# GPUPeople/spECK

Measured on AMD Instinct MI355X. Metric: SpGEMM GFLOP/s (2*flops_intermediate/s), A*A, higher is better.
Workload: dtype f64; 1 GPU; scircuit-like A*A (SURVEY 8d stand-in); rows=170998, nnzA=965730, products=8470902, nnzC=5291656, parallelism=single

## Files before the change

### speck_amd/csrc/esc_rows.hpp

```cpp
#pragma once
#include <type_traits>

#include "device_common.hpp"
#include "launch.hpp"
#include "row_groups.hpp"
#include "esc.hpp"

namespace speck {

template <typename T>
using Acc = double;

template <typename T, u32 L>
constexpr u32 num_esc_group_lds()
{
    return 4u * L * (u32)sizeof(Acc<T>) + L * (4u + (u32)sizeof(Acc<T>));
}

template <typename T, u32 L>
__device__ __forceinline__ u32 num_esc_row(const SubWave<L>& g, unsigned char* mine, const ProductSrc<T>& src, u32 a0, u32 a1,
                                           u32* __restrict__ out_col, T* __restrict__ out_val, u32 room)
{
    static_assert(L == 8 || L == 16, "8 or 16 lanes per row");
    using Mask = typename std::conditional<L <= 8, u32, u64>::type;
    constexpr u32 PER = kEscPerLane, NP = PER * L, TAG = L == 8 ? 5u : 6u;
    Acc<T>* s_vals = reinterpret_cast<Acc<T>*>(mine);
    Acc<T>* s_av = s_vals + NP;
    u32* s_off = reinterpret_cast<u32*>(s_av + L);
    const u32 gl = g.lane;
    const bool have = a0 + gl < a1;
    uint2 sl = make_uint2(0u, 0u);
    Acc<T> av = 0;
    if (have) {
        sl = src.b_sl[a0 + gl];
        av = (Acc<T>)src.a_val[a0 + gl];
    }
    u32 total;
    const u32 incl = g.inclusive_scan(sl.y, &total, nullptr);
    const bool nonempty = sl.y != 0;
    const u32 before = (u32)__popcll(g.ballot(nonempty) & ((1ull << gl) - 1ull));
    if (nonempty) {
        s_off[before] = sl.x - (incl - sl.y);
        s_av[before] = av;
    }
    Mask ends;
    if constexpr (L == 8) {
        ends = esc_group_or((nonempty && incl < 32u) ? (1u << incl) : 0u);
    } else {
        const u64 bit = (nonempty && incl < 64u) ? (1ull << incl) : 0ull;
        ends = (u64(esc_row_or((u32)(bit >> 32))) << 32) | esc_row_or((u32)bit);
    }
    wave_lds_fence();
    u32 key[PER], c[PER];
    T bv[PER];
    Acc<T> a[PER];
#pragma unroll
    for (u32 u = 0; u < PER; ++u) {
        const u32 p = u * L + gl;
        c[u] = 0;
        bv[u] = T(0);
        a[u] = 0;
        if (p < total) {
            u32 j;
            if constexpr (L <= 8) j = (u32)__popc(ends & ((2u << p) - 1u));
            else j = (u32)__popcll(ends & ((2ull << p) - 1ull));
            const u32 ib = s_off[j] + p;
            c[u] = src.b_col[ib];
            bv[u] = src.b_val[ib];
            a[u] = s_av[j];
        }
    }
#pragma unroll
    for (u32 u = 0; u < PER; ++u) {
        const u32 p = u * L + gl;
        key[u] = kEscInvalid;
        if (p < total) {
            const T prod = (T)a[u] * bv[u];
            s_vals[p] = (Acc<T>)prod;
            key[u] = (c[u] << TAG) | p;
        }
    }
    wave_lds_fence();
    esc_sort<L>(key, gl);
    u32 col[PER];
    Acc<T> sum[PER];
#pragma unroll
    for (u32 r = 0; r < PER; ++r) {
        const bool valid = gl * PER + r < total;
        col[r] = valid ? key[r] >> TAG : kEscInvalid;
// ... 8 lines not shown
        sum[r] += same ? sum[r - 1] : Acc<T>(0);
    }
    const u32 prev_col = dpp_move<kDppRowShr + 1>(kEscInvalid, col[PER - 1]);
    const bool cont = gl != 0 && col[0] != kEscInvalid && prev_col == col[0];
    Acc<T> chain = sum[PER - 1];
    bool stop = !(lead[PER - 1] && cont);
#pragma unroll
    for (u32 d = 1; d < L; d <<= 1) {
        Acc<T> t;
        bool ts;
        if (d == 1) {
            t = dpp_move_f64<kDppRowShr + 1>(0.0, chain);
            ts = dpp_move<kDppRowShr + 1>(1u, (u32)stop) != 0;
        } else if (d == 2) {
            t = dpp_move_f64<kDppRowShr + 2>(0.0, chain);
            ts = dpp_move<kDppRowShr + 2>(1u, (u32)stop) != 0;
        } else if (d == 4) {
            t = dpp_move_f64<kDppRowShr + 4>(0.0, chain);
            ts = dpp_move<kDppRowShr + 4>(1u, (u32)stop) != 0;
        } else {
            t = dpp_move_f64<kDppRowShr + 8>(0.0, chain);
            ts = dpp_move<kDppRowShr + 8>(1u, (u32)stop) != 0;
        }
        const bool in_group = gl >= d;
        if (!stop && in_group) chain += t;
        stop = stop || !in_group || ts;
    }
    const Acc<T> from_prev = dpp_move_f64<kDppRowShr + 1>(0.0, chain);
    const Acc<T> carry = cont ? from_prev : Acc<T>(0);
#pragma unroll
    for (u32 r = 0; r < PER; ++r) sum[r] += lead[r] ? carry : Acc<T>(0);
    const u32 next_col = dpp_move<kDppRowShl + 1>(kEscInvalid, col[0]);
    bool tail[PER];
    u32 ntail = 0;
#pragma unroll
    for (u32 r = 0; r < PER; ++r) {
        const u32 after = r + 1 < PER ? col[r + 1] : (gl == L - 1 ? kEscInvalid : next_col);
        tail[r] = col[r] != kEscInvalid && after != col[r];
        ntail += tail[r] ? 1u : 0u;
    }
    u32 all;
    u32 pos = g.inclusive_scan(ntail, &all, nullptr) - ntail;
    const bool write = all <= room;
#pragma unroll
    for (u32 r = 0; r < PER; ++r)
        if (tail[r] && write) {
            out_col[pos] = col[r];
            out_val[pos] = (T)sum[r];
            ++pos;
        }
    wave_lds_fence();
    return all;
}

template <typename T, u32 L, int THREADS, bool FUSED = false>
__device__ __forceinline__ void num_esc_body(unsigned char* smem, const ProductSrc<T>& src, const RowWork& w,
                                             u32* __restrict__ c_col, T* __restrict__ c_val, int cls, u32 bidx,
                                             u32 nblk, u32 hint = kNoCount, u32* __restrict__ counts = nullptr)
{
    using G = SubWave<L>;
    constexpr u32 NG = THREADS / L;
    const G g;
    const u32 gid = threadIdx.x / L;
    unsigned char* mine = smem + gid * num_esc_group_lds<T, L>();
    RowCursor cur = open_list<FUSED>(w, cls, hint, bidx, nblk, NG, gid, (w.xcd_aware & 8u) != 0);
    if (wave_void(cur.miss)) return;
    while (cur.more()) {
        const RowRec rec = cur.take();
        u32 place = rec.base, room = 0xFFFFFFFFu;
        if constexpr (FUSED) {
            place = w.nf_pred_off[rec.row];
            room = w.nf_pred_off[rec.row + 1] - place;
        }
        const u32 all = num_esc_row<T, L>(g, mine, src, rec.a0, rec.a1, c_col + place, c_val + place, room);
        if constexpr (FUSED) {
            if (g.lane == 0) {
                counts[rec.row] = all;
                if (all != room) const_cast<DeviceStats*>(w.st)->capacity_miss = 1;
            }
        }
    }
}

}
```

### speck_amd/csrc/esc_wide.hpp

```cpp
#pragma once
#include <type_traits>

#include "device_common.hpp"
#include "launch.hpp"
#include "row_groups.hpp"
#include "esc.hpp"
#include "esc_rows.hpp"

namespace speck {

constexpr int kDppRowRor8 = 0x128, kDppWaveShl1 = 0x130, kDppWaveShr1 = 0x138;

template <u32 M>
__device__ __forceinline__ u32 fetch_xor(u32 v)
{
    if constexpr (M == 1) return dpp_fetch<kDppQuadXor1>(v);
    else if constexpr (M == 2) return dpp_fetch<kDppQuadXor2>(v);
    else if constexpr (M == 3) return dpp_fetch<kDppQuadMirror>(v);
    else if constexpr (M == 4) return esc_xor4(v);
    else if constexpr (M == 7) return dpp_fetch<kDppRowHalfMirror>(v);
    else if constexpr (M == 8) return dpp_fetch<kDppRowRor8>(v);
    else {
        static_assert(M == 15, "lane masks inside a DPP row");
        return dpp_fetch<kDppRowMirror>(v);
// ... 59 lines not shown

template <u32 L>
__device__ __forceinline__ void esc_sort_wide(u32 (&x)[4], u32 gl)
{
    static_assert(L == 32 || L == 64, "32 or 64 lanes per row");
    esc_sort64(x, gl & 15u);
    esc_merge_stage<7>(x, gl);
    if constexpr (L == 64) esc_merge_stage<8>(x, gl);
}

template <int CTRL>
__device__ __forceinline__ double wave_move_f64(double fill, double v)
{
    return dpp_move_f64<CTRL>(fill, v);
}

template <u32 L>
struct EscEnds {
    static constexpr u32 NP = 4u * L, NW = NP / 32u;
    uint2* pref;
    template <class G>
    __device__ __forceinline__ void build(const G& g, bool nonempty, u32 incl) const
    {
        if (g.lane < NW) pref[g.lane].x = 0u;
        wave_lds_fence();
        if (nonempty && incl < NP) atomicOr(&pref[incl >> 5].x, 1u << (incl & 31u));
        wave_lds_fence();
        const u32 w = g.lane < NW ? pref[g.lane].x : 0u;
        const u32 pc = (u32)__popc(w);
        u32 total;
        const u32 inc = g.inclusive_scan(pc, &total, nullptr);
        if (g.lane < NW) pref[g.lane].y = inc - pc;
        wave_lds_fence();
    }
    __device__ __forceinline__ u32 owner(u32 p) const
    {
        const uint2 e = pref[p >> 5];
        return e.y + (u32)__popc(e.x & ((2u << (p & 31u)) - 1u));
    }
};

template <typename T, u32 L>
constexpr u32 num_escw_group_lds()
{
    return 4u * L * (u32)sizeof(Acc<T>) + L * ((u32)sizeof(Acc<T>) + 4u) + (4u * L / 32u) * 8u;
}
template <u32 L>
constexpr u32 sym_escw_group_lds()
{
    return L * 4u + (4u * L / 32u) * 8u;
}

template <typename T, u32 L>
__device__ __forceinline__ u32 num_escw_row(const SubWave<L>& g, unsigned char* mine, const ProductSrc<T>& src, u32 a0, u32 a1,
                                            u32 cmin, u32* __restrict__ out_col, T* __restrict__ out_val, u32 room)
{
    static_assert(L == 32 || L == 64, "32 or 64 lanes per row");
    constexpr u32 PER = kEscPerLane, NP = PER * L, TAG = L == 32 ? 7u : 8u;
    static_assert((1u << TAG) == NP, "the product number fills the tag");
    static_assert(TAG + (L == 32 ? kNumEsc32RangeBits : kNumEsc64RangeBits) == 32, "key = column offset << TAG | product");
    Acc<T>* s_vals = reinterpret_cast<Acc<T>*>(mine);
    Acc<T>* s_av = s_vals + NP;
    u32* s_off = reinterpret_cast<u32*>(s_av + L);
    const EscEnds<L> ends{reinterpret_cast<uint2*>(s_off + L)};
    const u32 gl = g.lane;
    const bool have = a0 + gl < a1;
    uint2 sl = make_uint2(0u, 0u);
    Acc<T> av = 0;
    if (have) {
        sl = src.b_sl[a0 + gl];
        av = (Acc<T>)src.a_val[a0 + gl];
    }
    u32 total;
    const u32 incl = g.inclusive_scan(sl.y, &total, nullptr);
    const bool nonempty = sl.y != 0;
    const u32 before = (u32)__popcll(g.ballot(nonempty) & ((1ull << gl) - 1ull));
    if (nonempty) {
        s_off[before] = sl.x - (incl - sl.y);
        s_av[before] = av;
    }
    ends.build(g, nonempty, incl);
    u32 key[PER], c[PER];
    T bv[PER];
    Acc<T> a[PER];
#pragma unroll
    for (u32 u = 0; u < PER; ++u) {
        const u32 p = u * L + gl;
        c[u] = 0;
        bv[u] = T(0);
        a[u] = 0;
        if (p < total) {
            const u32 j = ends.owner(p);
            const u32 ib = s_off[j] + p;
            c[u] = src.b_col[ib];
            bv[u] = src.b_val[ib];
            a[u] = s_av[j];
        }
    }
#pragma unroll
    for (u32 u = 0; u < PER; ++u) {
        const u32 p = u * L + gl;
        key[u] = kEscInvalid;
        if (p < total) {
            const T prod = (T)a[u] * bv[u];
            s_vals[p] = (Acc<T>)prod;
            key[u] = ((c[u] - cmin) << TAG) | p;
        }
    }
    wave_lds_fence();
    esc_sort_wide<L>(key, gl);
    u32 col[PER];
    Acc<T> sum[PER];
#pragma unroll
    for (u32 r = 0; r < PER; ++r) {
        const bool valid = gl * PER + r < total;
        col[r] = valid ? key[r] >> TAG : kEscInvalid;
        sum[r] = valid ? s_vals[key[r] & (NP - 1u)] : Acc<T>(0);
    }
    bool lead[PER];
    lead[0] = true;
#pragma unroll
    for (u32 r = 1; r < PER; ++r) {
        const bool same = col[r] == col[r - 1] && col[r] != kEscInvalid;
        lead[r] = lead[r - 1] && same;
        sum[r] += same ? sum[r - 1] : Acc<T>(0);
// ... 10 lines not shown
        const bool take = !stop && rl >= D_;                                     \
        chain += take ? t : Acc<T>(0);                                           \
        stop = take ? ts : stop;                                                 \
    }
    SPECK_SEG_ROW(1)
    SPECK_SEG_ROW(2)
    SPECK_SEG_ROW(4)
    SPECK_SEG_ROW(8)
#undef SPECK_SEG_ROW
    {
        const Acc<T> t = __longlong_as_double(
            (u64(dpp_move<kDppRowBcast15, 0xA>(0u, (u32)(__double_as_longlong(chain) >> 32))) << 32) |
            dpp_move<kDppRowBcast15, 0xA>(0u, (u32)__double_as_longlong(chain)));
        const bool ts = dpp_move<kDppRowBcast15, 0xA>(1u, (u32)stop) != 0;
        const bool take = !stop && (gl & 16u) != 0;
        chain += take ? t : Acc<T>(0);
        stop = take ? ts : stop;
    }
    if constexpr (L == 64) {
        const Acc<T> t = __longlong_as_double(
            (u64(dpp_move<kDppRowBcast31, 0xC>(0u, (u32)(__double_as_longlong(chain) >> 32))) << 32) |
            dpp_move<kDppRowBcast31, 0xC>(0u, (u32)__double_as_longlong(chain)));
        const bool ts = dpp_move<kDppRowBcast31, 0xC>(1u, (u32)stop) != 0;
        const bool take = !stop && (gl & 32u) != 0;
        chain += take ? t : Acc<T>(0);
        stop = take ? ts : stop;
    }
    const Acc<T> from_prev = wave_move_f64<kDppWaveShr1>(0.0, chain);
    const Acc<T> carry = cont ? from_prev : Acc<T>(0);
#pragma unroll
    for (u32 r = 0; r < PER; ++r) sum[r] += lead[r] ? carry : Acc<T>(0);
    const u32 next_col = dpp_move<kDppWaveShl1>(kEscInvalid, col[0]);
    bool tail[PER];
    u32 ntail = 0;
#pragma unroll
    for (u32 r = 0; r < PER; ++r) {
        const u32 after = r + 1 < PER ? col[r + 1] : (gl == L - 1 ? kEscInvalid : next_col);
        tail[r] = col[r] != kEscInvalid && after != col[r];
        ntail += tail[r] ? 1u : 0u;
    }
    u32 all;
    u32 pos = g.inclusive_scan(ntail, &all, nullptr) - ntail;
    const bool write = all <= room;
#pragma unroll
    for (u32 r = 0; r < PER; ++r)
        if (tail[r] && write) {
            out_col[pos] = col[r] + cmin;
            out_val[pos] = (T)sum[r];
            ++pos;
        }
    wave_lds_fence();
    return all;
}

template <typename T, u32 L, int THREADS, bool FUSED = false>
__device__ __forceinline__ void num_escw_body(unsigned char* smem, const ProductSrc<T>& src, const RowWork& w,
                                              u32* __restrict__ c_col, T* __restrict__ c_val, int cls, u32 bidx,
                                              u32 nblk, u32 hint = kNoCount, u32* __restrict__ counts = nullptr)
{
    using G = SubWave<L>;
    constexpr u32 NG = THREADS / L;
    const G g;
    const u32 gid = threadIdx.x / L;
    unsigned char* mine = smem + gid * num_escw_group_lds<T, L>();
    RowCursor cur = open_list<FUSED>(w, cls, hint, bidx, nblk, NG, gid, (w.xcd_aware & 8u) != 0);
    if (wave_void(cur.miss)) return;
    while (cur.more()) {
        const RowRec rec = cur.take();
        u32 place = rec.base, room = 0xFFFFFFFFu;
        if constexpr (FUSED) {
            place = w.nf_pred_off[rec.row];
            room = w.nf_pred_off[rec.row + 1] - place;
        }
        const u32 all = num_escw_row<T, L>(g, mine, src, rec.a0, rec.a1, rec.cmin, c_col + place, c_val + place, room);
        if constexpr (FUSED) {
            if (g.lane == 0) {
                counts[rec.row] = all;
                if (all != room) const_cast<DeviceStats*>(w.st)->capacity_miss = 1;
            }
        }
    }
}

template <u32 L, int THREADS>
__device__ __forceinline__ void sym_escw_body(unsigned char* smem, const ProductSrc<float>& src, const RowWork& w,
                                              u32* __restrict__ counts, int cls, u32 bidx, u32 nblk,
                                              u32 hint = kNoCount)
{
    static_assert(L == 32 || L == 64, "32 or 64 lanes per row");
    using G = SubWave<L>;
    constexpr u32 NG = THREADS / L, PER = kEscPerLane;
    const G g;
    const u32 gid = threadIdx.x / L;
    u32* s_off = reinterpret_cast<u32*>(smem + gid * sym_escw_group_lds<L>());
    const EscEnds<L> ends{reinterpret_cast<uint2*>(s_off + L)};
    RowCursor cur = open_list<true>(w, cls, hint, bidx, nblk, NG, gid, (w.xcd_aware & 8u) != 0);
    if (wave_void(cur.miss)) return;
    const u32 gl = g.lane;
    while (cur.more()) {
        const RowRec rec = cur.take();
        uint2 sl = make_uint2(0u, 0u);
        if (rec.a0 + gl < rec.a1) sl = src.b_sl[rec.a0 + gl];
        u32 total;
        const u32 incl = g.inclusive_scan(sl.y, &total, nullptr);
        const bool nonempty = sl.y != 0;
        const u32 before = (u32)__popcll(g.ballot(nonempty) & ((1ull << gl) - 1ull));
        if (nonempty) s_off[before] = sl.x - (incl - sl.y);
        ends.build(g, nonempty, incl);
        u32 col[PER];
#pragma unroll
        for (u32 u = 0; u < PER; ++u) {
            const u32 p = u * L + gl;
            col[u] = kEscInvalid;
            if (p < total) col[u] = src.b_col[s_off[ends.owner(p)] + p];
        }
        esc_sort_wide<L>(col, gl);
        const u32 prev_col = dpp_move<kDppWaveShr1>(kEscInvalid, col[PER - 1]);
        u32 heads = 0;
#pragma unroll
        for (u32 r = 0; r < PER; ++r) {
            const u32 before_col = r ? col[r - 1] : (gl ? prev_col : kEscInvalid);
            heads += (col[r] != kEscInvalid && col[r] != before_col) ? 1u : 0u;
        }
        heads = g.reduce_add(heads, nullptr);
        if (gl == 0) store_row_count(w, counts, rec.row, heads);
        wave_lds_fence();
    }
}

}
```

### speck_amd/csrc/launch.hpp

```cpp
#pragma once
#include <hip/hip_ext.h>

#include "chain.hpp"
#include "device_common.hpp"

namespace speck {

u32 analysis_blocks(u32 m);
void set_analysis_wide_rows(u32 avg_len);
u32 scan_tiles(u32 m);

constexpr u32 kListRegions = (((u32)SYM_CLASSES > (u32)NUM_CLASSES ? (u32)SYM_CLASSES : (u32)NUM_CLASSES) + 1u) / 2u;
__host__ __device__ inline size_t class_list_records(u32 m) { return size_t(kListRegions) * (m ? m : 1u); }
template <typename Rec>
__host__ __device__ __forceinline__ Rec* class_rec_at(Rec* lists, u32 m, u32 cls, u32 i)
{
    return two_sided_at(lists, m, cls, i);
}

void launch_analysis(hipStream_t s, const u32* a_ro, const u32* a_col, const u32* b_ro, const u32* b_col, u32 m, u64 nnz_a,
                     u32* row_ops, u32* row_max_ops, u32* row_col_min, u32* row_col_max, u8* sym_cls, u32* counts,
                     RowRec* sym_recs, DeviceStats* st, const ClassifyParams& cp, uint2* b_sl, const Chain& chain,
                     u64* nf_off = nullptr, u64 expect_nf = ~0ull, u32 b_rows = ~0u,
                     u32* a_ro_copy = nullptr ,
// ... 213 lines not shown
void note_launch_status(hipError_t e, const char* what);
int take_launch_error();
#define SPECK_LAUNCH(kernel_, ...)                                          \
    do {                                                                    \
        hipLaunchKernelGGL(kernel_, __VA_ARGS__);                           \
        ::speck::note_launch_status(hipGetLastError(), #kernel_);           \
    } while (0)
#define SPECK_LAUNCH_TIMED(kernel_, grid_, block_, lds_, stream_, e0_, e1_, ...)                            \
    do {                                                                                                   \
        if (e0_) hipExtLaunchKernelGGL(kernel_, grid_, block_, lds_, stream_, e0_, e1_, 0, __VA_ARGS__);   \
        else hipLaunchKernelGGL(kernel_, grid_, block_, lds_, stream_, __VA_ARGS__);                       \
        ::speck::note_launch_status(hipGetLastError(), #kernel_);                                          \
    } while (0)

template <typename T>
void launch_numeric(hipStream_t s, int cls, u32 count, const CsrView<T>& A, const CsrView<T>& B,
                    const RowWork& w, u32* c_col, T* c_val, int cu_count);

template <typename T>
void launch_walk(hipStream_t s, const WalkArgs& args, const ProductSrc<T>& src, const Chain& chain, hipEvent_t e0 = nullptr,
                 hipEvent_t e1 = nullptr);

u32 grid_for(u32 count, u32 lds, int threads, int cu_count, u32 rows_per_block);

template <typename K>
void set_dyn_lds(K kernel, u32 bytes)
{
    if (bytes > 48 * 1024)
        note_launch_status(hipFuncSetAttribute(reinterpret_cast<const void*>(kernel),
                                               hipFuncAttributeMaxDynamicSharedMemorySize, (int)bytes),
                           "hipFuncSetAttribute(MaxDynamicSharedMemorySize)");
}

template <size_t N, typename LdsFn>
bool plan_light(const ClassSlot (&tab)[N], u32 mask, const u32* counts_hint, bool exact, int cu_count, LdsFn&& class_lds,
                u32 extra, hipStream_t s, hipEvent_t e0, hipEvent_t e1, ClassGrid* cg, u32* lds)
{
    *lds = 0;
    for (const ClassSlot& t : tab)
        if (mask >> t.cls & 1u) *lds = *lds > class_lds(t.cls) ? *lds : class_lds(t.cls);
    *cg = ClassGrid{};
    for (size_t k = 0; k < N; ++k) {
        const u32 hint = counts_hint[tab[k].cls];
        const bool on = (mask >> tab[k].cls & 1u) && hint;
        cg->first[k + 1] = cg->first[k] + (on ? grid_for(hint, *lds, 256, cu_count, tab[k].rows) : 0u);
        cg->cnt[k] = exact ? hint : kNoCount;
    }
    cg->first[N + 1] = cg->first[N] + extra;
    if (cg->first[N + 1] != 0) return true;
    if (e0) (void)hipEventRecord(e0, s), (void)hipEventRecord(e1, s);
    return false;
}
void set_grid_rounds(u32 block_classes, u32 subwave_classes);
void set_b8k_full_first(u32 mask);
void set_scan_small_items(int items);
void set_spill_big_grid(u32 blocks);

u32 symbolic_lds_bytes(int cls);
u32 numeric_lds_bytes(int cls, u32 vsize);

}
```

### speck_amd/csrc/numeric.hip

```cpp
#include <algorithm>
#include <type_traits>

#include "chain3.hpp"
#include "device_common.hpp"
#include "launch.hpp"
#include "row_groups.hpp"
#include "esc_rows.hpp"
#include "esc_wide.hpp"

namespace speck {

template <typename T, int THREADS>
constexpr u32 num_direct_lds()
{
    return THREADS * (12u + (u32)sizeof(T)) + (THREADS / 64 + 2 + win_words<Block<THREADS>>() + 3) / 4 * 16;
}

template <typename T, int THREADS>
__device__ __forceinline__ void num_direct_body(unsigned char* smem, const ProductSrc<T>& src, const RowWork& w,
                                                u32* __restrict__ c_col, T* __restrict__ c_val, u32 bidx,
                                                u32 nblk, u32 hint = kNoCount)
{
    using G = Block<THREADS>;
    const G g;
// ... 1552 lines not shown
void set_b8k_full_first(u32 mask) { g_b8k_full_first = mask; }
static u32 g_spill_big_grid = 256;
void set_spill_big_grid(u32 blocks) { g_spill_big_grid = blocks ? blocks : 256u; }

template <typename T, bool VERIFY>
static void launch_b8k(hipStream_t s, u32 count, const ProductSrc<T>& A, const u32* B, const RowWork& w, u32* c_col,
                       T* c_val, int cu_count)
{
    constexpr int cls = NUM_B8K;
    if (w.sliced) {
        const u32 sl = num_sliced_lds(num_group_lds<Block<256>, T, kNumB2KCap, 256>());
        SPECK_LAUNCH((num_sliced_kernel<T, VERIFY>), dim3(grid_for(count, sl, 256, cu_count, 1)), dim3(256), sl, s, A, B, w,
                     c_col, c_val, cls);
        return;
    }
    const auto all = launch_num_hash<Block<512>, T, kNumB8KCap, kB8KW1, kNumB8KMaxNnz, SORT_BITMAP, 512, 0, VERIFY>;
    const auto upper = launch_num_hash<Block<512>, T, kNumB8KCap, kB8KW1, kNumB8KMaxNnz, SORT_BITMAP, 512, kNumB8KHalfMaxNnz, VERIFY>;
    const auto lower = launch_num_hash<Block<512>, T, kNumB8KCap / 2, kB8KW1, kNumB8KHalfMaxNnz, SORT_BITMAP, 512, 0, VERIFY>;
    if (count * 2 < (u32)cu_count) {
        all(s, cls, count, A, B, w, c_col, c_val, cu_count);
        return;
    }
    const bool full_first = (g_b8k_full_first & (VERIFY ? 2u : 1u)) != 0;
    if (full_first) upper(s, cls, count, A, B, w, c_col, c_val, cu_count);
    lower(s, cls, count, A, B, w, c_col, c_val, cu_count);
    if (!full_first) upper(s, cls, count, A, B, w, c_col, c_val, cu_count);
}

template <typename T, bool VERIFY>
static void launch_d2(hipStream_t s, u32 count, const ProductSrc<T>& A, const u32* B, const RowWork& w, u32* c_col,
                      T* c_val, int cu_count)
{
    auto k = num_dense_kernel<T, kNumD2Cols, 1024, VERIFY>;
    const u32 lds = numeric_lds_bytes_t<T>(NUM_D2);
    set_dyn_lds(k, lds);
    SPECK_LAUNCH(k, dim3(grid_for(count, lds, 1024, cu_count, 1)), dim3(1024), lds, s, A, B, w, c_col, c_val, (int)NUM_D2);
}

template <typename T>
void launch_numeric_light(hipStream_t s, const u32* counts_hint, u32 mask, const CsrView<T>& Av,
                          const CsrView<T>& Bv, const RowWork& w, u32* c_col, T* c_val, int cu_count, bool exact,
                          hipEvent_t e0, hipEvent_t e1)
{
    constexpr size_t NS = kNumLightSlots;
    const u32 off_blocks = w.off_n ? std::min<u32>((w.off_n + 2047u) / 2048u, 512u) : 0u;
    ClassGrid cg;
    u32 lds;
    if (!plan_light(kNumLight, mask, counts_hint, exact, cu_count, numeric_lds_bytes_t<T>, off_blocks, s, e0, e1, &cg, &lds)) return;
    const bool tiny_only = cg.first[kNumTinyFirst] == 0 && !w.verify_numeric && !w.off_n;
    const ProductSrc<T> src{w.b_sl, Av.data, Bv.col_ids, Bv.data, w.w_sl};
    bool with_esc = false;
    for (size_t k = 0; k < NS; ++k)
        if ((kNumEscMask >> kNumLight[k].cls & 1u) && cg.first[k + 1] != cg.first[k]) with_esc = true;
    if (w.verify_numeric)
        SPECK_LAUNCH_TIMED((num_light_kernel<T, false, true>), dim3(cg.first[NS + 1]), dim3(256), lds, s, e0, e1, src,
                           Av.row_offsets, w, c_col, c_val, cg);
    else if (!tiny_only && with_esc)
        SPECK_LAUNCH_TIMED((num_light_kernel<T, true>), dim3(cg.first[NS + 1]), dim3(256), lds, s, e0, e1, src, Av.row_offsets, w,
                           c_col, c_val, cg);
    else if (!tiny_only)
        SPECK_LAUNCH_TIMED((num_light_kernel<T, false>), dim3(cg.first[NS + 1]), dim3(256), lds, s, e0, e1, src, Av.row_offsets, w,
                           c_col, c_val, cg);
    else
        SPECK_LAUNCH_TIMED((num_tiny_kernel<T>), dim3(cg.first[NS]), dim3(256), lds, s, e0, e1, src, Av.row_offsets, w,
                           c_col, c_val, cg);
}

template <typename T>
void launch_numeric_first(hipStream_t s, u32 count, const CsrView<T>& Av, const CsrView<T>& Bv, const RowWork& w,
                          u32* counts, int cu_count, u32 wcols, hipEvent_t e0, hipEvent_t e1)
{
    if (count == 0) {
        if (e0) (void)hipEventRecord(e0, s), (void)hipEventRecord(e1, s);
        return;
    }
    const ProductSrc<T> src{w.b_sl, Av.data, Bv.col_ids, Bv.data, w.w_sl};
    wcols = wcols < 256u ? 256u : (wcols > kNumD1Cols ? kNumD1Cols : (wcols + 255u) & ~255u);
    const u32 lds = (wcols + 256) * (u32)sizeof(Acc<T>) + wcols +
                    (2 * 256 + 256 / 64 + 2 + win_words<Block<256>>() + 3) / 4 * 16;
    if (w.nf_pred_off) {
        set_dyn_lds((nf_dense_kernel<T, 256, true>), lds);
        SPECK_LAUNCH_TIMED((nf_dense_kernel<T, 256, true>), dim3(grid_for(count, lds, 256, cu_count, 1)), dim3(256), lds, s, e0,
                           e1, src, Av.row_offsets, w, counts, wcols);
        return;
    }
    set_dyn_lds((nf_dense_kernel<T, 256>), lds);
    SPECK_LAUNCH_TIMED((nf_dense_kernel<T, 256>), dim3(grid_for(count, lds, 256, cu_count, 1)), dim3(256), lds, s, e0, e1,
                       src, Av.row_offsets, w, counts, wcols);
}

template <typename T>
void launch_numeric(hipStream_t s, int cls, u32 count, const CsrView<T>& Av, const CsrView<T>& Bv,
                    const RowWork& w, u32* c_col, T* c_val, int cu_count)
{
    if (count == 0) return;
    const ProductSrc<T> A{w.b_sl, Av.data, Bv.col_ids, Bv.data, w.w_sl};
    const u32* B = Av.row_offsets;
    switch (cls) {
        case NUM_B8K:
            if (w.verify_numeric)
                launch_b8k<T, true>(s, count, A, B, w, c_col, c_val, cu_count);
            else
                launch_b8k<T, false>(s, count, A, B, w, c_col, c_val, cu_count);
            break;
        case NUM_D2:
            if (w.verify_numeric)
// ... 71 lines not shown
```

### speck_amd/csrc/pipeline.hip

```cpp
#include <hip/hip_runtime.h>

#include <algorithm>
#include <chrono>
#include <cstdio>
#include <cstdlib>
#include <cstring>
#include <string>
#include <vector>

#include "../../include/speck_c_api.h"
#include "chain3.hpp"
#include "host_common.hpp"
#include "launch.hpp"
#include "row_groups.hpp"
#include "masked.hpp"
#include "select.hpp"
#include "add.hpp"
#include "scale.hpp"
#include "sort_rows.hpp"
#include "tile_scratch.hpp"
#include "coo.hpp"
#include "extract.hpp"
#include "topk.hpp"
#include "sample.hpp"
// ... 1888 lines not shown
        c->prev.valid = false;
        c->sort.release();
        c->masked.release();
        c->select.release();
        c->add.release();
        c->reduce.release();
        c->scale.release();
        c->spmv.release();
        c->spmm.release();
        c->sddmm.release();
        c->softmax.release();
        c->spmm_t.release();
        c->coo.release();
        c->extract.release();
        c->topk.release();
        c->sample.release();
    }
    else if (n == "sort_reg_max") c->sort.reg_max = (u32)std::min<int64_t>(std::max<int64_t>(value, 0), SPECK_SORT_REG_MAX);
    else if (n == "sort_lds_max") c->sort.lds_max = (u32)std::min<int64_t>(std::max<int64_t>(value, 0), SPECK_SORT_LDS_MAX);
    else if (n == "topk_group_max") c->topk.group_max = (u32)std::min<int64_t>(std::max<int64_t>(value, 0), SPECK_TOPK_GROUP_MAX);
    else if (n == "topk_lds_max") c->topk.lds_max = (u32)std::min<int64_t>(std::max<int64_t>(value, 0), SPECK_TOPK_LDS_MAX);
    else if (n == "sample_group_max") c->sample.group_max = (u32)std::min<int64_t>(std::max<int64_t>(value, 0), SPECK_SAMPLE_GROUP_MAX);
    else if (n == "sample_lds_max") c->sample.lds_max = (u32)std::min<int64_t>(std::max<int64_t>(value, 0), SPECK_SAMPLE_LDS_MAX);
    else if (n == "mask_group_max") c->masked.group_max = (u32)std::min<int64_t>(std::max<int64_t>(value, 0), SPECK_MASK_GROUP_MAX);
    else if (n == "mask_lds_max") c->masked.lds_max = (u32)std::min<int64_t>(std::max<int64_t>(value, 0), SPECK_MASK_LDS_MAX);
    else if (n == "walk_debug") set_walk_debug((u32)value & 0xFFFFu, (u32)(value >> 16));
    else if (n == "verify_inputs") c->verify_inputs = value != 0, c->snap_for_arena = false, forget(false);
    else if (n == "num_verify") c->num_verify = (int)value, forget(false);
    else if (n == "skip_scan") c->skip_scan = value != 0, forget(false);
    else if (n == "overlap_analysis") c->overlap_analysis = value != 0, forget(false);
    else if (n == "esc_fused") c->esc_fused = value != 0, forget(true);
    else if (n == "nf_direct") c->nf_direct = value != 0, forget(false);
    else if (n == "sym_w128") c->cp.sym_w128 = value != 0, forget(true);
    else if (n == "sym_g8") c->cp.sym_g8 = value != 0, forget(true);
    else if (n == "esc16") c->cp.esc16 = value != 0, forget(true);
    else if (n == "slice_rows") c->cp.slice_ops = value ? kSliceMaxOps : 0u, forget(true);
    else if (n == "esc32") c->cp.esc32 = value != 0, forget(true);
    else if (n == "esc64") c->cp.esc64 = value != 0, forget(true);
    else if (n == "num_g8") c->cp.num_g8 = value != 0, forget(true);
    else if (n == "num_w256") c->cp.num_w256 = value != 0, forget(true);
    else if (n == "collect_bytes") c->cp.want_bytes = value != 0;
    else if (n == "concurrent_classes") c->concurrent_classes = value != 0;
    else if (n == "validate_inputs") c->validate_inputs = value != 0;
    else if (n == "validate_after_nnz") c->validate_after_nnz = (u64)value;
    else if (n == "spin_wait") c->spin_wait = value != 0, forget(false);
    else if (n == "fork_min_us") c->fork_min_us = (float)value, forget(false);
    else if (n == "max_side_streams") c->max_side_streams = (u32)value, forget(false);
    else if (n == "reuse" || n == "use_graph") {
        if (c->reuse != (value != 0)) forget(true);
        c->reuse = value != 0;
    }
    else if (n == "grid_rounds_block") set_grid_rounds((u32)value, 0), forget(false);
    else if (n == "grid_rounds_sub") set_grid_rounds(0, (u32)value), forget(false);
    else if (n == "spill_big_grid") set_spill_big_grid((u32)value), forget(false);
    else if (n == "scan_small_items") set_scan_small_items((int)value), forget(true);
    else if (n == "b8k_full_first") set_b8k_full_first((u32)value), forget(false);
    else if (n == "xcd_aware") c->xcd_aware = (u32)value, forget(false);
    else return SPECK_ERR_INVALID;
    return SPECK_OK;
}

int speck_config_profile_kernels(speck_config* c, int enable)
{
    if (!c) return SPECK_ERR_INVALID;
    c->profile_kernels = enable == 2 ? 2 : (enable != 0 ? 1 : 0);
    return SPECK_OK;
}

int speck_last_stats(const speck_config* c, speck_stats* out)
{
    if (!c || !out) return SPECK_ERR_INVALID;
    *out = c->last;
    out->numeric_reruns = c->replay_misses;
    out->graph_replays = c->replays;
    out->graph_captures = c->plans_made;
    out->pool_fallbacks = c->pool_fallbacks;
    out->scratch_pool_bytes = c->nfpool_bytes;
    out->walk_misses = c->walk_misses;
    return SPECK_OK;
}

static int check_guards(speck_config* c, const speck_dcsr* C, int rc)
{
    if (!guard_bytes() || !c) return rc;
    std::vector<GuardZone> inner = c->arena_zones;
    inner.insert(inner.end(), c->gpool_zones.begin(), c->gpool_zones.end());
    inner.insert(inner.end(), c->nfpool_zones.begin(), c->nfpool_zones.end());
    const void* whole[] = {c->arena, c->snap, c->pred.off, c->gpred.off, c->nfpool, c->gpool,
                           C ? C->data : nullptr, C ? C->col_ids : nullptr, C ? C->row_offsets : nullptr};
    static const char* names[] = {"arena", "input snapshot", "row-offset copy", "row-offset copy (sequence)", "scratch pool",
                                  "spill pool", "C.data", "C.col_ids", "C.row_offsets"};
    return guard_check_buffers(whole, names, 9, main_stream(c), nullptr, rc, std::move(inner));
}

int speck_multiply_f64(speck_config* c, const speck_dcsr* A, const speck_dcsr* B, speck_dcsr* C,
                       speck_timings* t)
{
    return check_guards(c, C, multiply_impl<double>(c, A, B, C, t));
}

int speck_multiply_f32(speck_config* c, const speck_dcsr* A, const speck_dcsr* B, speck_dcsr* C,
                       speck_timings* t)
{
    return check_guards(c, C, multiply_impl<float>(c, A, B, C, t));
}

// ... 137 lines not shown
```

### speck_amd/csrc/symbolic.hip

```cpp
#include "device_common.hpp"
#include "launch.hpp"
#include "row_groups.hpp"
#include "esc.hpp"
#include "esc_rows.hpp"
#include "esc_wide.hpp"

namespace speck {

template <class G, int THREADS>
constexpr u32 sym_scratch_words()
{
    return G::kIsBlock ? (THREADS / 64 + 2) : 0;
}

template <class G, u32 CAP, int THREADS>
constexpr u32 sym_group_lds()
{
    return (CAP + 2 * G::SIZE + sym_scratch_words<G, THREADS>() + win_words<G>() + 3u) / 4u * 16u;
}

template <class G, u32 CAP, int THREADS>
__device__ __forceinline__ void sym_hash_body(unsigned char* smem, const ProductSrc<float>& src,
                                              const RowWork& w, u32* __restrict__ counts, int cls, u32 bidx,
                                              u32 nblk, u32 hint = kNoCount)
{
    constexpr u32 NG = THREADS / G::SIZE;
    constexpr u32 kGroupBytes = sym_group_lds<G, CAP, THREADS>();
    const G g;
    const u32 gid = G::kIsBlock ? 0u : threadIdx.x / G::SIZE;
    u32* tab = reinterpret_cast<u32*>(smem + gid * kGroupBytes);
    u32* scratch = tab + CAP + 2 * G::SIZE;
    RowMeta<float> meta{tab + CAP, tab + CAP + G::SIZE, nullptr, scratch + sym_scratch_words<G, THREADS>()};
    RowCursor cur = open_list<true>(w, cls, hint, bidx, nblk, NG, gid, (w.xcd_aware & (G::kIsBlock ? 4u : 1u)) != 0);
    if (group_void(g, cur.miss)) return;
    while (cur.more()) {
        const RowRec rec = cur.take();
        static_assert(CAP % (4 * G::SIZE) == 0, "the key set is cleared 16 bytes per lane and step");
        for (u32 q = g.lane; q < CAP / 4; q += G::SIZE)
            reinterpret_cast<uint4*>(tab)[q] = make_uint4(kEmptyKey, kEmptyKey, kEmptyKey, kEmptyKey);
        g.sync();
        u32 cnt = 0;
        for_each_product<false>(g, src, rec.a0, rec.a1, meta, scratch,
                                [&](const u32(&c)[kBatch], const float(&)[kBatch], u32 n) {
                                    cnt += set_insert_batch<CAP>(tab, c, n);
                                });
        cnt = g.reduce_add(cnt, scratch);
        if (g.lane == 0) store_row_count(w, counts, rec.row, cnt);
        g.sync();
    }
}

template <u32 L>
constexpr u32 sym_esc_group_lds() { return L * 4u; }

template <u32 L, int THREADS>
__device__ __forceinline__ void sym_esc_body(unsigned char* smem, const ProductSrc<float>& src, const RowWork& w,
                                             u32* __restrict__ counts, int cls, u32 bidx, u32 nblk,
                                             u32 hint = kNoCount)
{
    using G = SubWave<L>;
    constexpr u32 NG = THREADS / L, PER = kEscPerLane;
    const G g;
    const u32 gid = threadIdx.x / L;
    u32* s_off = reinterpret_cast<u32*>(smem + gid * sym_esc_group_lds<L>());
    RowCursor cur = open_list<true>(w, cls, hint, bidx, nblk, NG, gid, (w.xcd_aware & 8u) != 0);
    if (wave_void(cur.miss)) return;
    const u32 gl = g.lane;
    while (cur.more()) {
        const RowRec rec = cur.take();
        uint2 sl = make_uint2(0u, 0u);
        if (rec.a0 + gl < rec.a1) sl = src.b_sl[rec.a0 + gl];
        u32 total;
        const u32 incl = g.inclusive_scan(sl.y, &total, nullptr);
        const bool nonempty = sl.y != 0;
        const u32 before = (u32)__popcll(g.ballot(nonempty) & ((1ull << gl) - 1ull));
        if (nonempty) s_off[before] = sl.x - (incl - sl.y);
        u64 ends;
        if constexpr (L == 8) {
            ends = esc_group_or((nonempty && incl < 32u) ? (1u << incl) : 0u);
        } else {
            const u64 bit = (nonempty && incl < 64u) ? (1ull << incl) : 0ull;
            ends = (u64(esc_row_or((u32)(bit >> 32))) << 32) | esc_row_or((u32)bit);
        }
        wave_lds_fence();
        u32 col[PER];
#pragma unroll
        for (u32 u = 0; u < PER; ++u) {
            const u32 p = u * L + gl;
            col[u] = kEscInvalid;
            if (p < total) col[u] = src.b_col[s_off[(u32)__popcll(ends & ((2ull << p) - 1ull))] + p];
        }
        esc_sort<L>(col, gl);
        const u32 prev_col = dpp_move<kDppRowShr + 1>(kEscInvalid, col[PER - 1]);
        u32 heads = 0;
#pragma unroll
        for (u32 r = 0; r < PER; ++r) {
            const u32 before_col = r ? col[r - 1] : (gl ? prev_col : kEscInvalid);
            heads += (col[r] != kEscInvalid && col[r] != before_col) ? 1u : 0u;
        }
        heads = g.reduce_add(heads, nullptr);
        if (gl == 0) store_row_count(w, counts, rec.row, heads);
        wave_lds_fence();
    }
}

template <u32 WORDS, int THREADS>
__device__ __forceinline__ void sym_bitmap_body(unsigned char* smem, const ProductSrc<float>& src,
                                                const RowWork& w, u32* __restrict__ counts, int cls, u32 bidx,
                                                u32 nblk, u32 hint = kNoCount)
{
    using G = Block<THREADS>;
    const G g;
    u32* bm = reinterpret_cast<u32*>(smem);
    u32* scratch = bm + WORDS + 2 * THREADS;
    RowMeta<float> meta{bm + WORDS, bm + WORDS + THREADS, nullptr, scratch + THREADS / 64 + 2};
    constexpr u64 kWindowCols = u64(WORDS) * 32;
    RowCursor cur = open_list<true>(w, cls, hint, bidx, nblk, 1u, 0u, (w.xcd_aware & 2u) != 0);
    if (block_void(cur.miss)) return;
    while (cur.more()) {
        const RowRec rec = cur.take();
        u32 total = 0;
        const bool multi = u64(rec.cmax) - rec.cmin + 1 > kWindowCols;
        const WindowCursors<THREADS> cur{src.b_sl, src.b_col, src.w_sl, rec.a0, rec.a1};
        ProductSrc<float> wsrc = src;
        if (multi) {
            wsrc.b_sl = src.w_sl;
            cur.reset();
        }
        u32 base = rec.cmin;
        while (true) {
            if (multi) {
                base = cur.next_window((u32)kWindowCols, scratch);
                if (base == 0xFFFFFFFFu) break;
            }
            const u64 left = u64(rec.cmax) - base + 1;
            const u32 ncols = left < kWindowCols ? (u32)left : (u32)kWindowCols;
            const u32 nwords = (ncols + 31) >> 5;
            for (u32 i = threadIdx.x; i < nwords; i += THREADS) bm[i] = 0;
            __syncthreads();
            for_each_product<false>(g, wsrc, rec.a0, rec.a1, meta, scratch,
                                    [&](const u32(&c)[kBatch], const float(&)[kBatch], u32 n) {
#pragma unroll
                                        for (int u = 0; u < kBatch; ++u) {
                                            const u32 d = c[u] - base;
                                            bitmap_or_runs(bm, ((u32)u < n && d < ncols) ? d >> 5 : 0xFFFFFFFFu, 1u << (d & 31));
                                        }
                                    });
            for (u32 i = threadIdx.x; i < nwords; i += THREADS) total += __popc(bm[i]);
            __syncthreads();
            if (!multi) break;
        }
        total = g.reduce_add(total, scratch);
        if (threadIdx.x == 0) store_row_count(w, counts, rec.row, total);
    }
}
// ... 148 lines not shown
    else if (b < cg.first[3])
        sym_hash_body<SubWave<64>, kSymW1KCap, 256>(smem, src, w, counts, SYM_W1K, b - cg.first[2], cg.first[3] - cg.first[2], cg.cnt[2]);
    else if (b < cg.first[4])
        sym_hash_body<SubWave<32>, kSymW256Cap, 256>(smem, src, w, counts, SYM_W256, b - cg.first[3], cg.first[4] - cg.first[3], cg.cnt[3]);
    else if (b < cg.first[5])
        num_escw_body<T, 64, 256, true>(smem, nsrc, w, w.nf_direct_col, static_cast<T*>(w.nf_direct_val), SYM_R64,
                                        b - cg.first[4], cg.first[5] - cg.first[4], cg.cnt[4], counts);
    else if (b < cg.first[6])
        num_escw_body<T, 32, 256, true>(smem, nsrc, w, w.nf_direct_col, static_cast<T*>(w.nf_direct_val), SYM_R32,
                                        b - cg.first[5], cg.first[6] - cg.first[5], cg.cnt[5], counts);
    else if (b < cg.first[7])
        sym_hash_body<SubWave<16>, kSymW128Cap, 256>(smem, src, w, counts, SYM_W128, b - cg.first[6], cg.first[7] - cg.first[6], cg.cnt[6]);
    else if (b < cg.first[8])
        num_esc_body<T, 16, 256, true>(smem, nsrc, w, w.nf_direct_col, static_cast<T*>(w.nf_direct_val), SYM_G16,
                                       b - cg.first[7], cg.first[8] - cg.first[7], cg.cnt[7], counts);
    else
        num_esc_body<T, 8, 256, true>(smem, nsrc, w, w.nf_direct_col, static_cast<T*>(w.nf_direct_val), SYM_G8,
                                      b - cg.first[8], cg.first[9] - cg.first[8], cg.cnt[8], counts);
}

u32 symbolic_lds_bytes(int cls)
{
    const u32 groups = class_rows(kSymLight, cls);
    static_assert(class_rows(kSymLight, SYM_G8) == 256 / 8 && class_rows(kSymLight, SYM_G16) == 256 / 16 &&
                      class_rows(kSymLight, SYM_R32) == 256 / 32 && class_rows(kSymLight, SYM_R64) == 256 / 64 &&
                      class_rows(kSymLight, SYM_W128) == 256 / 16 && class_rows(kSymLight, SYM_W256) == 256 / 32 &&
                      class_rows(kSymLight, SYM_W1K) == 256 / 64,
                  "rows per workgroup = 256 threads / the lanes of the class' group (the bodies in sym_light_kernel)");
    switch (cls) {
        case SYM_G8: return groups * sym_esc_group_lds<8>();
        case SYM_G16: return groups * sym_esc_group_lds<16>();
        case SYM_R32: return groups * sym_escw_group_lds<32>();
        case SYM_R64: return groups * sym_escw_group_lds<64>();
        case SYM_W128: return groups * sym_group_lds<SubWave<16>, kSymW128Cap, 256>();
        case SYM_W256: return groups * sym_group_lds<SubWave<32>, kSymW256Cap, 256>();
        case SYM_W1K: return groups * sym_group_lds<SubWave<64>, kSymW1KCap, 256>();
        case SYM_B4K: return sym_group_lds<Block<256>, kSymB4KCap, 256>();
        case SYM_B16K: return sym_group_lds<Block<512>, kSymB16KCap, 512>();
        case SYM_B32K: return sym_group_lds<Block<1024>, kSymB32KCap, 1024>();
        case SYM_BM1: return (kSymBm1Words + 2 * 256 + 8 + win_words<Block<256>>()) * 4;
        case SYM_BM2: return (kSymBm2Words + 2 * 1024 + 24 + win_words<Block<1024>>()) * 4;
        case SYM_GH: return (2 * kGhThreads + kGhThreads / 64 + 8 + win_words<Block<kGhThreads>>()) * 4;
    }
    return 0;
}

static u32 g_grid_rounds_block = 1, g_grid_rounds_sub = 4;
void set_grid_rounds(u32 block_classes, u32 subwave_classes)
{
    if (block_classes) g_grid_rounds_block = block_classes;
    if (subwave_classes) g_grid_rounds_sub = subwave_classes;
}

u32 grid_for(u32 count, u32 lds, int threads, int cu_count, u32 rows_per_block)
{
    u32 per_cu = lds ? (160u * 1024u) / lds : 8;
    const u32 by_threads = 2048u / (u32)threads;
    if (per_cu > by_threads) per_cu = by_threads;
    if (per_cu < 1) per_cu = 1;
    u32 rounds = rows_per_block > 1 ? g_grid_rounds_sub : g_grid_rounds_block;
    if (rows_per_block == 1 && g_grid_rounds_block == 1 && lds <= 48u * 1024u) rounds = 16;
    const u64 cap = u64(cu_count) * per_cu * rounds;
    u64 need = (u64(count) + rows_per_block - 1) / rows_per_block;
    if (need > cap) need = cap;
    return need ? (u32)need : 1u;
}

template <class G, u32 CAP, int THREADS>
static void launch_sym_hash(hipStream_t s, int cls, u32 count, const ProductSrc<float>& A,
                            const u32* B, const RowWork& w, u32* counts, int cu_count)
{
    auto k = sym_hash_kernel<G, CAP, THREADS>;
    const u32 lds = symbolic_lds_bytes(cls);
    set_dyn_lds(k, lds);
    SPECK_LAUNCH(k, dim3(grid_for(count, lds, THREADS, cu_count, THREADS / G::SIZE)),
                       dim3(THREADS), lds, s, A, B, w, counts, cls);
}

void launch_symbolic_light(hipStream_t s, const u32* counts_hint, u32 mask, const u32* a_ro,
                           const uint2* b_sl, const u32* b_col, const RowWork& w,
                           u32* counts, int cu_count, bool exact, u32 fused_vsize, const void* a_val,
                           const void* b_val, hipEvent_t e0, hipEvent_t e1)
{
    constexpr size_t NS = kSymLightSlots;
    const bool fused = fused_vsize != 0 && (mask & kSymEscMask) != 0;
    auto class_lds = [&](int cls) -> u32 {
        return fused && fused_num_class(cls) >= 0 ? numeric_lds_bytes(fused_num_class(cls), fused_vsize) : symbolic_lds_bytes(cls);
    };
    ClassGrid cg;
    u32 lds;
    if (!plan_light(kSymLight, mask, counts_hint, exact, cu_count, class_lds, 0u, s, e0, e1, &cg, &lds)) return;
    if (fused && fused_vsize == 8) {
        const ProductSrc<double> nsrc{b_sl, static_cast<const double*>(a_val), b_col, static_cast<const double*>(b_val), w.w_sl};
        SPECK_LAUNCH_TIMED((sym_light_fused_kernel<double>), dim3(cg.first[NS]), dim3(256), lds, s, e0, e1, nsrc, a_ro, w, counts, cg);
        return;
    }
    if (fused) {
        const ProductSrc<float> nsrc{b_sl, static_cast<const float*>(a_val), b_col, static_cast<const float*>(b_val), w.w_sl};
        SPECK_LAUNCH_TIMED((sym_light_fused_kernel<float>), dim3(cg.first[NS]), dim3(256), lds, s, e0, e1, nsrc, a_ro, w, counts, cg);
        return;
    }
    const ProductSrc<float> src{b_sl, nullptr, b_col, nullptr, w.w_sl};
    SPECK_LAUNCH_TIMED(sym_light_kernel, dim3(cg.first[NS]), dim3(256), lds, s, e0, e1, src, a_ro, w, counts, cg);
}

void launch_symbolic(hipStream_t s, int cls, u32 count, const u32* a_ro, const uint2* b_sl,
                     const u32* b_col, const RowWork& w, u32* counts, int cu_count)
{
    if (count == 0) return;
    const ProductSrc<float> A{b_sl, nullptr, b_col, nullptr, w.w_sl};
    const u32* B = a_ro;
    const u32 lds = symbolic_lds_bytes(cls);
    switch (cls) {
        case SYM_B16K: launch_sym_hash<Block<512>, kSymB16KCap, 512>(s, cls, count, A, B, w, counts, cu_count); break;
        case SYM_B32K: launch_sym_hash<Block<1024>, kSymB32KCap, 1024>(s, cls, count, A, B, w, counts, cu_count); break;
        case SYM_BM2: {
            auto k = sym_bitmap_kernel<kSymBm2Words, 1024>;
            set_dyn_lds(k, lds);
            SPECK_LAUNCH(k, dim3(grid_for(count, lds, 1024, cu_count, 1)), dim3(1024), lds, s, A,
                               B, w, counts, cls);
            break;
        }
        case SYM_GH:
            SPECK_LAUNCH(sym_global_hash_kernel, dim3(grid_for(count, lds, kGhThreads, cu_count, 1)),
                               dim3(kGhThreads), lds, s, A, B, w, counts);
            break;
        default:
            note_launch_status(hipErrorInvalidValue, "launch_symbolic: not a heavy class");
    }
}

}
```

Measured before the change: 134.7 GFLOP/s.

## Prefetch next row's A entries in ESC loops and stretch ESC grid walks

The ESC row loops in the numeric and symbolic subwave kernels now issue the global loads for the next row's B slice descriptors and A values before processing the current row. This hides the load latency behind the current row's sort and scan. The light-class grid is also resized with a new stretch_walks step, which caps the ESC block count near a queried occupancy so each subwave walks several rows and has something to prefetch. The cost is extra registers, a possible occupancy drop, and fewer blocks, which can hurt load balance.

```diff
diff --git a/speck_amd/csrc/esc_rows.hpp b/speck_amd/csrc/esc_rows.hpp
--- a/speck_amd/csrc/esc_rows.hpp
+++ b/speck_amd/csrc/esc_rows.hpp
@@ -17,9 +17,39 @@
     return 4u * L * (u32)sizeof(Acc<T>) + L * (4u + (u32)sizeof(Acc<T>));
 }
 
+template <typename T>
+struct EscEntry {
+    uint2 sl;
+    T av;
+};
+template <typename T>
+__device__ __forceinline__ uint2 esc_request_sl(const ProductSrc<T>& src, u32 a0, u32 a1, u32 gl, bool there = true)
+{
+    uint2 sl = make_uint2(0u, 0u);
+    if (there && a0 + gl < a1) sl = src.b_sl[a0 + gl];
+    return sl;
+}
+template <typename T>
+__device__ __forceinline__ EscEntry<T> esc_request(const ProductSrc<T>& src, u32 a0, u32 a1, u32 gl, bool there = true)
+{
+    EscEntry<T> e{make_uint2(0u, 0u), T(0)};
+    if (there && a0 + gl < a1) {
+        e.sl = src.b_sl[a0 + gl];
+        e.av = src.a_val[a0 + gl];
+    }
+    return e;
+}
+__device__ __forceinline__ void esc_settle(uint2& sl) { asm volatile("" : "+v"(sl.x), "+v"(sl.y)); }
+template <typename T>
+__device__ __forceinline__ void esc_settle(EscEntry<T>& e)
+{
+    asm volatile("" : "+v"(e.sl.x), "+v"(e.sl.y), "+v"(e.av));
+}
+
 template <typename T, u32 L>
-__device__ __forceinline__ u32 num_esc_row(const SubWave<L>& g, unsigned char* mine, const ProductSrc<T>& src, u32 a0, u32 a1,
-                                           u32* __restrict__ out_col, T* __restrict__ out_val, u32 room)
+__device__ __forceinline__ u32 num_esc_row(const SubWave<L>& g, unsigned char* mine, const ProductSrc<T>& src,
+                                           const EscEntry<T>& mine_a, u32* __restrict__ out_col, T* __restrict__ out_val,
+                                           u32 room)
 {
     static_assert(L == 8 || L == 16, "8 or 16 lanes per row");
     using Mask = typename std::conditional<L <= 8, u32, u64>::type;
@@ -28,13 +58,8 @@
     Acc<T>* s_av = s_vals + NP;
     u32* s_off = reinterpret_cast<u32*>(s_av + L);
     const u32 gl = g.lane;
-    const bool have = a0 + gl < a1;
-    uint2 sl = make_uint2(0u, 0u);
-    Acc<T> av = 0;
-    if (have) {
-        sl = src.b_sl[a0 + gl];
-        av = (Acc<T>)src.a_val[a0 + gl];
-    }
+    const uint2 sl = mine_a.sl;
+    const Acc<T> av = (Acc<T>)mine_a.av;
     u32 total;
     const u32 incl = g.inclusive_scan(sl.y, &total, nullptr);
     const bool nonempty = sl.y != 0;
@@ -149,6 +174,12 @@
     wave_lds_fence();
     return all;
 }
+template <typename T, u32 L>
+__device__ __forceinline__ u32 num_esc_row(const SubWave<L>& g, unsigned char* mine, const ProductSrc<T>& src, u32 a0, u32 a1,
+                                           u32* __restrict__ out_col, T* __restrict__ out_val, u32 room)
+{
+    return num_esc_row<T, L>(g, mine, src, esc_request(src, a0, a1, g.lane), out_col, out_val, room);
+}
 
 template <typename T, u32 L, int THREADS, bool FUSED = false>
 __device__ __forceinline__ void num_esc_body(unsigned char* smem, const ProductSrc<T>& src, const RowWork& w,
@@ -162,15 +193,26 @@
     unsigned char* mine = smem + gid * num_esc_group_lds<T, L>();
     RowCursor cur = open_list<FUSED>(w, cls, hint, bidx, nblk, NG, gid, (w.xcd_aware & 8u) != 0);
     if (wave_void(cur.miss)) return;
-    while (cur.more()) {
-        const RowRec rec = cur.take();
-        u32 place = rec.base, room = 0xFFFFFFFFu;
-        if constexpr (FUSED) {
-            place = w.nf_pred_off[rec.row];
-            room = w.nf_pred_off[rec.row + 1] - place;
-        }
-        const u32 all = num_esc_row<T, L>(g, mine, src, rec.a0, rec.a1, c_col + place, c_val + place, room);
-        if constexpr (FUSED) {
+    if constexpr (!FUSED) {
+        bool have = cur.more();
+        RowRec rec = cur.take();
+        EscEntry<T> ea = esc_request(src, rec.a0, rec.a1, g.lane, have);
+        esc_settle(ea);
+        while (have) {
+            const bool succ = cur.more();
+            const EscEntry<T> en = esc_request(src, cur.next.a0, cur.next.a1, g.lane, succ);
+            const RowRec nrec = cur.take();
+            num_esc_row<T, L>(g, mine, src, ea, c_col + rec.base, c_val + rec.base, 0xFFFFFFFFu);
+            ea = en;
+            rec = nrec;
+            have = succ;
+        }
+    } else {
+        while (cur.more()) {
+            const RowRec rec = cur.take();
+            const u32 place = w.nf_pred_off[rec.row];
+            const u32 room = w.nf_pred_off[rec.row + 1] - place;
+            const u32 all = num_esc_row<T, L>(g, mine, src, rec.a0, rec.a1, c_col + place, c_val + place, room);
             if (g.lane == 0) {
                 counts[rec.row] = all;
                 if (all != room) const_cast<DeviceStats*>(w.st)->capacity_miss = 1;
diff --git a/speck_amd/csrc/esc_wide.hpp b/speck_amd/csrc/esc_wide.hpp
--- a/speck_amd/csrc/esc_wide.hpp
+++ b/speck_amd/csrc/esc_wide.hpp
@@ -135,8 +135,9 @@
 }
 
 template <typename T, u32 L>
-__device__ __forceinline__ u32 num_escw_row(const SubWave<L>& g, unsigned char* mine, const ProductSrc<T>& src, u32 a0, u32 a1,
-                                            u32 cmin, u32* __restrict__ out_col, T* __restrict__ out_val, u32 room)
+__device__ __forceinline__ u32 num_escw_row(const SubWave<L>& g, unsigned char* mine, const ProductSrc<T>& src,
+                                            const EscEntry<T>& mine_a, u32 cmin, u32* __restrict__ out_col,
+                                            T* __restrict__ out_val, u32 room)
 {
     static_assert(L == 32 || L == 64, "32 or 64 lanes per row");
     constexpr u32 PER = kEscPerLane, NP = PER * L, TAG = L == 32 ? 7u : 8u;
@@ -147,13 +148,8 @@
     u32* s_off = reinterpret_cast<u32*>(s_av + L);
     const EscEnds<L> ends{reinterpret_cast<uint2*>(s_off + L)};
     const u32 gl = g.lane;
-    const bool have = a0 + gl < a1;
-    uint2 sl = make_uint2(0u, 0u);
-    Acc<T> av = 0;
-    if (have) {
-        sl = src.b_sl[a0 + gl];
-        av = (Acc<T>)src.a_val[a0 + gl];
-    }
+    const uint2 sl = mine_a.sl;
+    const Acc<T> av = (Acc<T>)mine_a.av;
     u32 total;
     const u32 incl = g.inclusive_scan(sl.y, &total, nullptr);
     const bool nonempty = sl.y != 0;
@@ -270,6 +266,12 @@
     wave_lds_fence();
     return all;
 }
+template <typename T, u32 L>
+__device__ __forceinline__ u32 num_escw_row(const SubWave<L>& g, unsigned char* mine, const ProductSrc<T>& src, u32 a0, u32 a1,
+                                            u32 cmin, u32* __restrict__ out_col, T* __restrict__ out_val, u32 room)
+{
+    return num_escw_row<T, L>(g, mine, src, esc_request(src, a0, a1, g.lane), cmin, out_col, out_val, room);
+}
 
 template <typename T, u32 L, int THREADS, bool FUSED = false>
 __device__ __forceinline__ void num_escw_body(unsigned char* smem, const ProductSrc<T>& src, const RowWork& w,
@@ -283,15 +285,26 @@
     unsigned char* mine = smem + gid * num_escw_group_lds<T, L>();
     RowCursor cur = open_list<FUSED>(w, cls, hint, bidx, nblk, NG, gid, (w.xcd_aware & 8u) != 0);
     if (wave_void(cur.miss)) return;
-    while (cur.more()) {
-        const RowRec rec = cur.take();
-        u32 place = rec.base, room = 0xFFFFFFFFu;
-        if constexpr (FUSED) {
-            place = w.nf_pred_off[rec.row];
-            room = w.nf_pred_off[rec.row + 1] - place;
-        }
-        const u32 all = num_escw_row<T, L>(g, mine, src, rec.a0, rec.a1, rec.cmin, c_col + place, c_val + place, room);
-        if constexpr (FUSED) {
+    if constexpr (!FUSED) {
+        bool have = cur.more();
+        RowRec rec = cur.take();
+        EscEntry<T> ea = esc_request(src, rec.a0, rec.a1, g.lane, have);
+        esc_settle(ea);
+        while (have) {
+            const bool succ = cur.more();
+            const EscEntry<T> en = esc_request(src, cur.next.a0, cur.next.a1, g.lane, succ);
+            const RowRec nrec = cur.take();
+            num_escw_row<T, L>(g, mine, src, ea, rec.cmin, c_col + rec.base, c_val + rec.base, 0xFFFFFFFFu);
+            ea = en;
+            rec = nrec;
+            have = succ;
+        }
+    } else {
+        while (cur.more()) {
+            const RowRec rec = cur.take();
+            const u32 place = w.nf_pred_off[rec.row];
+            const u32 room = w.nf_pred_off[rec.row + 1] - place;
+            const u32 all = num_escw_row<T, L>(g, mine, src, rec.a0, rec.a1, rec.cmin, c_col + place, c_val + place, room);
             if (g.lane == 0) {
                 counts[rec.row] = all;
                 if (all != room) const_cast<DeviceStats*>(w.st)->capacity_miss = 1;
@@ -315,10 +328,14 @@
     RowCursor cur = open_list<true>(w, cls, hint, bidx, nblk, NG, gid, (w.xcd_aware & 8u) != 0);
     if (wave_void(cur.miss)) return;
     const u32 gl = g.lane;
-    while (cur.more()) {
-        const RowRec rec = cur.take();
-        uint2 sl = make_uint2(0u, 0u);
-        if (rec.a0 + gl < rec.a1) sl = src.b_sl[rec.a0 + gl];
+    bool have = cur.more();
+    RowRec rec = cur.take();
+    uint2 sl = esc_request_sl(src, rec.a0, rec.a1, gl, have);
+    esc_settle(sl);
+    while (have) {
+        const bool succ = cur.more();
+        const uint2 sn = esc_request_sl(src, cur.next.a0, cur.next.a1, gl, succ);
+        const RowRec nrec = cur.take();
         u32 total;
         const u32 incl = g.inclusive_scan(sl.y, &total, nullptr);
         const bool nonempty = sl.y != 0;
@@ -343,7 +360,10 @@
         heads = g.reduce_add(heads, nullptr);
         if (gl == 0) store_row_count(w, counts, rec.row, heads);
         wave_lds_fence();
-    }
-}
-
-}
+        sl = sn;
+        rec = nrec;
+        have = succ;
+    }
+}
+
+}
diff --git a/speck_amd/csrc/launch.hpp b/speck_amd/csrc/launch.hpp
--- a/speck_amd/csrc/launch.hpp
+++ b/speck_amd/csrc/launch.hpp
@@ -289,6 +289,29 @@
     return false;
 }
 void set_grid_rounds(u32 block_classes, u32 subwave_classes);
+void set_esc_walk(u32 rows, int64_t resident_override);
+u32 esc_walk_rows();
+template <size_t N>
+void stretch_walks(const ClassSlot (&tab)[N], u32 esc_mask, u32 resident, ClassGrid* cg)
+{
+    const u32 R = esc_walk_rows();
+    u64 esc = 0;
+    for (size_t k = 0; k < N; ++k)
+        if (esc_mask >> tab[k].cls & 1u) esc += cg->first[k + 1] - cg->first[k];
+    const u64 others = cg->first[N + 1] - esc;
+    const u64 room = resident - (others < resident / 2 ? others : resident / 2);
+    if (R <= 1 || esc <= room) return;
+    u32 need[N + 1];
+    for (size_t k = 0; k <= N; ++k) need[k] = cg->first[k + 1] - cg->first[k];
+    for (size_t k = 0; k < N; ++k) {
+        if (!(esc_mask >> tab[k].cls & 1u) || !need[k]) continue;
+        const u64 share = room * need[k] / esc, by_rows = (u64(need[k]) + R - 1) / R;
+        const u64 blocks = share > by_rows ? share : by_rows;
+        need[k] = blocks ? (u32)blocks : 1u;
+    }
+    for (size_t k = 0; k <= N; ++k) cg->first[k + 1] = cg->first[k] + need[k];
+}
+u32 light_resident(const void* kernel, u32 lds, int cu_count);
 void set_b8k_full_first(u32 mask);
 void set_scan_small_items(int items);
 void set_spill_big_grid(u32 blocks);
diff --git a/speck_amd/csrc/numeric.hip b/speck_amd/csrc/numeric.hip
--- a/speck_amd/csrc/numeric.hip
+++ b/speck_amd/csrc/numeric.hip
@@ -1628,6 +1628,11 @@
     bool with_esc = false;
     for (size_t k = 0; k < NS; ++k)
         if ((kNumEscMask >> kNumLight[k].cls & 1u) && cg.first[k + 1] != cg.first[k]) with_esc = true;
+    if (with_esc && !w.verify_numeric && esc_walk_rows() > 1) {
+        const void* k = tiny_only ? reinterpret_cast<const void*>(num_tiny_kernel<T>)
+                                  : reinterpret_cast<const void*>(num_light_kernel<T, true>);
+        stretch_walks(kNumLight, kNumEscMask, light_resident(k, lds, cu_count), &cg);
+    }
     if (w.verify_numeric)
         SPECK_LAUNCH_TIMED((num_light_kernel<T, false, true>), dim3(cg.first[NS + 1]), dim3(256), lds, s, e0, e1, src,
                            Av.row_offsets, w, c_col, c_val, cg);
diff --git a/speck_amd/csrc/pipeline.hip b/speck_amd/csrc/pipeline.hip
--- a/speck_amd/csrc/pipeline.hip
+++ b/speck_amd/csrc/pipeline.hip
@@ -1964,6 +1964,8 @@
     }
     else if (n == "grid_rounds_block") set_grid_rounds((u32)value, 0), forget(false);
     else if (n == "grid_rounds_sub") set_grid_rounds(0, (u32)value), forget(false);
+    else if (n == "esc_walk_rows") set_esc_walk((u32)std::max<int64_t>(value, 1), -1), forget(false);
+    else if (n == "esc_walk_resident") set_esc_walk(0, std::max<int64_t>(value, 0)), forget(false);
     else if (n == "spill_big_grid") set_spill_big_grid((u32)value), forget(false);
     else if (n == "scan_small_items") set_scan_small_items((int)value), forget(true);
     else if (n == "b8k_full_first") set_b8k_full_first((u32)value), forget(false);
diff --git a/speck_amd/csrc/symbolic.hip b/speck_amd/csrc/symbolic.hip
--- a/speck_amd/csrc/symbolic.hip
+++ b/speck_amd/csrc/symbolic.hip
@@ -66,10 +66,14 @@
     RowCursor cur = open_list<true>(w, cls, hint, bidx, nblk, NG, gid, (w.xcd_aware & 8u) != 0);
     if (wave_void(cur.miss)) return;
     const u32 gl = g.lane;
-    while (cur.more()) {
-        const RowRec rec = cur.take();
-        uint2 sl = make_uint2(0u, 0u);
-        if (rec.a0 + gl < rec.a1) sl = src.b_sl[rec.a0 + gl];
+    bool have = cur.more();
+    RowRec rec = cur.take();
+    uint2 sl = esc_request_sl(src, rec.a0, rec.a1, gl, have);
+    esc_settle(sl);
+    while (have) {
+        const bool succ = cur.more();
+        const uint2 sn = esc_request_sl(src, cur.next.a0, cur.next.a1, gl, succ);
+        const RowRec nrec = cur.take();
         u32 total;
         const u32 incl = g.inclusive_scan(sl.y, &total, nullptr);
         const bool nonempty = sl.y != 0;
@@ -101,6 +105,9 @@
         heads = g.reduce_add(heads, nullptr);
         if (gl == 0) store_row_count(w, counts, rec.row, heads);
         wave_lds_fence();
+        sl = sn;
+        rec = nrec;
+        have = succ;
     }
 }
 
@@ -355,6 +362,35 @@
     if (subwave_classes) g_grid_rounds_sub = subwave_classes;
 }
 
+static u32 g_esc_walk_rows = 4, g_esc_walk_resident = 0;
+void set_esc_walk(u32 rows, int64_t resident_override)
+{
+    if (rows) g_esc_walk_rows = rows;
+    if (resident_override >= 0) g_esc_walk_resident = (u32)resident_override;
+}
+u32 esc_walk_rows() { return g_esc_walk_rows; }
+
+u32 light_resident(const void* kernel, u32 lds, int cu_count)
+{
+    if (g_esc_walk_resident) return g_esc_walk_resident;
+    struct Known {
+        const void* kernel;
+        u32 lds, per_cu;
+    };
+    thread_local Known known[8];
+    thread_local u32 n_known = 0;
+    for (u32 i = 0; i < n_known; ++i)
+        if (known[i].kernel == kernel && known[i].lds == lds) return known[i].per_cu * (u32)cu_count;
+    int per_cu = 0;
+    if (hipOccupancyMaxActiveBlocksPerMultiprocessor(&per_cu, kernel, 256, lds) != hipSuccess || per_cu < 1) {
+        (void)hipGetLastError();
+        per_cu = lds ? (int)std::min<u32>(160u * 1024u / lds, 8u) : 8;
+        if (per_cu < 1) per_cu = 1;
+    }
+    if (n_known < 8) known[n_known++] = Known{kernel, lds, (u32)per_cu};
+    return (u32)per_cu * (u32)cu_count;
+}
+
 u32 grid_for(u32 count, u32 lds, int threads, int cu_count, u32 rows_per_block)
 {
     u32 per_cu = lds ? (160u * 1024u) / lds : 8;
@@ -404,6 +440,8 @@
         return;
     }
     const ProductSrc<float> src{b_sl, nullptr, b_col, nullptr, w.w_sl};
+    if (esc_walk_rows() > 1)
+        stretch_walks(kSymLight, kSymEscMask, light_resident(reinterpret_cast<const void*>(sym_light_kernel), lds, cu_count), &cg);
     SPECK_LAUNCH_TIMED(sym_light_kernel, dim3(cg.first[NS]), dim3(256), lds, s, e0, e1, src, a_ro, w, counts, cg);
 }
 
```

Result: faster. 137.3 GFLOP/s, median of 6 (+1.9%).
